# distributed-information-bottleneck/distributed-information-bottleneck.github.io

Hardware: AMD Instinct MI355X
Metric: DIB train samples/sec (fwd+KL+bwd+Adam) (higher is better)
Workload: dtype f32; 1 GPU; BASELINE config 3: synthetic tabular, 2^20 rows x 64 scalar features resident in HBM, posenc [2,4,8,16], encoder [128,128], E=32, integration [256,256], out=1, BCE-from-logits, Adam; per_gpu_batch=65536, global_batch=65536, parallelism=dp1, rccl_ranks_joined=1, dataset_rows=1048576, params=2224897

## Files before the change

distributed-information-bottleneck.github.io_amd/csrc/dib_api.hip:

```cpp
#include <algorithm>
#include <atomic>
#include <cmath>
#include <cstdio>
#include <cstdlib>
#include <cstring>
#include <map>
#include <mutex>
#include <new>
#include <utility>
#include <vector>

#include "../../include/dib_hip.h"
#include "dib_elementwise.h"
#include "dib_gauss_lse.h"
#include "dib_mi_rows.h"
#include "dib_gemm.h"
#include "dib_wgrad_stream.h"
#include "dib_infonce_mfma.h"
#include "dib_fused.h"
#include "dib_wgrad_recompute.h"
#include "dib_tail.h"
#include "dib_small.h"
#include "dib_st.h"
#include "dib_attn.h"
#include "dib_attn_small.h"
#include "dib_st_chain.h"
#include "dib_measure.h"
#include "dib_circuit.h"
#include "dib_partition.h"
#include "dib_st_info.h"
#include "dib_mi_channel.h"
#include "dib_input_grad.h"
#include "../../include/dib_st.h"
#include "../../include/dib_measure.h"
#include "../../include/dib_circuit.h"
#include "../../include/dib_partition.h"
#include "../../include/dib_mi_channel.h"

#include "host/common.h"
#include "host/layout.h"
#include "host/gemm.h"
#include "host/encoder.h"
#include "host/input_grad.h"
#include "host/small.h"
#include "host/step.h"
#include "host/infonce.h"
#include "host/st.h"
#include "host/mi.h"
#include "host/measure.h"
#include "host/circuit.h"
#include "host/partition.h"
```

distributed-information-bottleneck.github.io_amd/csrc/host/common.h:

```cpp

static std::atomic<unsigned long long> g_dib_launches{0};
#define DIB_LAUNCH(...) do { g_dib_launches.fetch_add(1, std::memory_order_relaxed); hipLaunchKernelGGL(__VA_ARGS__); } while (0)

namespace {

constexpr int64_t kAlign = 64;
constexpr int kMaxSplits = 32;
constexpr int kSmallMaxBatch = 2048;
constexpr int kSmallMaxEncWgs = 1024;
constexpr size_t kSmallMaxLds = 160 * 1024;
constexpr int kSplitRows = 512;
inline int64_t align_up(int64_t v, int64_t a = kAlign) { return (v + a - 1) / a * a; }
inline int cdiv(int64_t a, int64_t b) { return (int)((a + b - 1) / b); }
inline int grid_for(int64_t n, int per_block = 256, int cap = 256 * 16) {
  return (int)std::max<int64_t>(1, std::min<int64_t>((n + per_block - 1) / per_block, cap));
}

constexpr int kProfCats = 19;
constexpr int kProfWgradH1Part = 19;
constexpr int kProfFusedFwd = 12, kProfFusedBwd = 13, kProfOther = 14, kProfAttnFwd = 15, kProfAttnBwd = 16;
constexpr int kProfWgradStream128 = 17, kProfWgradStream64 = 18;
struct Prof {
  std::atomic<bool> on{false};
  std::mutex mu;
  std::vector<hipEvent_t> pool;
  std::vector<std::pair<hipEvent_t, hipEvent_t>> spans[kProfCats];
  std::vector<size_t> h1_spans;
  hipEvent_t get() {
    if (!pool.empty()) { hipEvent_t e = pool.back(); pool.pop_back(); return e; }
    hipEvent_t e = nullptr;
    (void)hipEventCreate(&e);
    return e;
  }
} g_prof;

struct ProfScope {
  int cat; hipStream_t st; hipEvent_t a = nullptr, b = nullptr;
  bool h1_part;
  ProfScope(int c, hipStream_t s, bool h1 = false) : cat(c), st(s), h1_part(h1) {
    if (g_prof.on.load(std::memory_order_relaxed) && cat != 14) {
      { std::lock_guard<std::mutex> lk(g_prof.mu); a = g_prof.get(); b = g_prof.get(); }
      (void)hipEventRecord(a, st);
    }
  }
  ~ProfScope() {
    if (a) {
      (void)hipEventRecord(b, st);
      std::lock_guard<std::mutex> lk(g_prof.mu);
      if (h1_part) g_prof.h1_spans.push_back(g_prof.spans[cat].size());
      g_prof.spans[cat].push_back({a, b});
    }
  }
};

const char* kVersion = "dib_hip 0.4 (gfx950: fused encoder-bank fwd/bwd + grouped fp32-MFMA GEMM + flash attention)";

int act_ok(int a) { return a >= 0 && a <= 7; }

struct Tuning {
  int fwd_small_wgs = 512;
  int fwd_narrow_wgs = 1024;
  int stream_rows = 8192;
  int split_policy = 1;
  int split_overhead = 128;
  int fused_encoder = 1;
  int fused_head = 1;
  int small_batch = 1;
  int small_wgs = 512;
  int mlp_row_tiles = 1;
  int infonce_one_launch = 1;
  int attn_small_bwd_waves = 8;
  int wgrad_flat_tile = 1;
  int wgrad_stream = 1;
  int wgrad_stream_rows = 8192;
  int wgrad_stream_fill = 85;
  int wgrad_recompute_h1 = 1;
  int attn_fwd_waves = 8;
  int int_cluster_short_exchange = 1;
  int int_cluster = 8;
  int int_cluster_wgs = 256;
  int int_cluster_min_weights = 65536;
  int wgrad_max_splits = 32;
  int num_cus = 0;
};
inline Tuning& tuning() { static Tuning t; return t; }
inline const Tuning& knobs() { return tuning(); }
inline int wgrad_max_splits() { return std::max(1, std::min(32, knobs().wgrad_max_splits)); }
inline int device_cus() {
  static std::atomic<int> cus[64];
  int dev = 0;
  if (hipGetDevice(&dev) != hipSuccess || dev < 0 || dev >= 64) return 256;
  int v = cus[dev].load(std::memory_order_relaxed);
  if (v > 0) return v;
  if (hipDeviceGetAttribute(&v, hipDeviceAttributeMultiprocessorCount, dev) != hipSuccess || v <= 0) return 256;
  cus[dev].store(v, std::memory_order_relaxed);
  return v;
}
inline int split_rule_cus() { return knobs().num_cus > 0 ? knobs().num_cus : device_cus(); }

std::mutex g_attr_mu;
template <auto* Kernel>
int raise_dynamic_lds(size_t bytes) {
  if (bytes <= 64 * 1024) return DIB_OK;
  static std::atomic<size_t> granted[64];
  int dev = 0;
  std::atomic<size_t>* slot = hipGetDevice(&dev) == hipSuccess && dev >= 0 && dev < 64 ? &granted[dev] : nullptr;
  if (slot && slot->load(std::memory_order_acquire) >= bytes) return DIB_OK;
  std::lock_guard<std::mutex> lk(g_attr_mu);
  if (slot && slot->load(std::memory_order_relaxed) >= bytes) return DIB_OK;
  hipError_t e = hipFuncSetAttribute((const void*)Kernel, hipFuncAttributeMaxDynamicSharedMemorySize, (int)bytes);
  if (e != hipSuccess) return (int)e;
  if (slot) slot->store(bytes, std::memory_order_release);
  return DIB_OK;
}
template <auto* Kernel, typename... Args>
int launch_lds(dim3 grid, dim3 block, size_t lds, hipStream_t st, Args&&... args) {
  if (int rc = raise_dynamic_lds<Kernel>(lds)) return rc;
  DIB_LAUNCH(Kernel, grid, block, lds, st, std::forward<Args>(args)...);
  return (int)hipGetLastError();
}

static int* tuning_slot(const char* key) {
  Tuning& t = tuning();
  if (!key) return nullptr;
  if (!std::strcmp(key, "fwd_small_wgs")) return &t.fwd_small_wgs;
  if (!std::strcmp(key, "fwd_narrow_wgs")) return &t.fwd_narrow_wgs;
  if (!std::strcmp(key, "stream_rows")) return &t.stream_rows;
  if (!std::strcmp(key, "split_policy")) return &t.split_policy;
  if (!std::strcmp(key, "split_overhead")) return &t.split_overhead;
  if (!std::strcmp(key, "fused_encoder")) return &t.fused_encoder;
  if (!std::strcmp(key, "fused_head")) return &t.fused_head;
  if (!std::strcmp(key, "small_batch")) return &t.small_batch;
  if (!std::strcmp(key, "small_wgs")) return &t.small_wgs;
  if (!std::strcmp(key, "mlp_row_tiles")) return &t.mlp_row_tiles;
  if (!std::strcmp(key, "infonce_one_launch")) return &t.infonce_one_launch;
  if (!std::strcmp(key, "attn_small_bwd_waves")) return &t.attn_small_bwd_waves;
  if (!std::strcmp(key, "wgrad_flat_tile")) return &t.wgrad_flat_tile;
  if (!std::strcmp(key, "wgrad_stream")) return &t.wgrad_stream;
  if (!std::strcmp(key, "wgrad_stream_rows")) return &t.wgrad_stream_rows;
  if (!std::strcmp(key, "wgrad_stream_fill")) return &t.wgrad_stream_fill;
  if (!std::strcmp(key, "wgrad_recompute_h1")) return &t.wgrad_recompute_h1;
  if (!std::strcmp(key, "wgrad_max_splits")) return &t.wgrad_max_splits;
  if (!std::strcmp(key, "num_cus")) return &t.num_cus;
  if (!std::strcmp(key, "attn_fwd_waves")) return &t.attn_fwd_waves;
  if (!std::strcmp(key, "int_cluster_short_exchange")) return &t.int_cluster_short_exchange;
  if (!std::strcmp(key, "int_cluster")) return &t.int_cluster;
  if (!std::strcmp(key, "int_cluster_wgs")) return &t.int_cluster_wgs;
  if (!std::strcmp(key, "int_cluster_min_weights")) return &t.int_cluster_min_weights;
  return nullptr;
}

}

extern "C" {

const char* dib_version(void) { return kVersion; }
int dib_abi_version(void) { return DIB_ABI_VERSION; }

const char* dib_error_string(int code) {
  switch (code) {
    case DIB_OK: return "ok";
    case DIB_E_ARG: return "invalid argument";
    case DIB_E_SHAPE: return "shape mismatch";
    case DIB_E_WORKSPACE: return "workspace / descriptor tables missing";
    case DIB_E_UNSUPPORTED: return "unsupported configuration";
    case DIB_E_NODEVICE: return "no HIP device";
    default: return code > 0 ? hipGetErrorString((hipError_t)code) : "unknown dib error";
  }
}

int dib_set_tuning(const char* key, int value) {
  int* p = tuning_slot(key);
  if (!p || value < 0) return DIB_E_ARG;
  *p = value;
  return DIB_OK;
}

int dib_get_tuning(const char* key, int* value) {
  const int* p = tuning_slot(key);
  if (!p || !value) return DIB_E_ARG;
  *value = *p;
  return DIB_OK;
}

int64_t dib_launch_count(void) { return (int64_t)g_dib_launches.load(std::memory_order_relaxed); }

int dib_profile_enable(int on) {
  std::lock_guard<std::mutex> lk(g_prof.mu);
  for (int c = 0; c < kProfCats; ++c) {
    for (auto& sp : g_prof.spans[c]) { g_prof.pool.push_back(sp.first); g_prof.pool.push_back(sp.second); }
    g_prof.spans[c].clear();
  }
  g_prof.h1_spans.clear();
  g_prof.on = on != 0;
  return DIB_OK;
}

int dib_profile_summary_n(double* ms_by_category, int* launches_by_category, int n) {
  if (!ms_by_category || !launches_by_category || n < 0) return DIB_E_ARG;
  std::lock_guard<std::mutex> lk(g_prof.mu);
  for (int c = 0; c < std::min(n, kProfCats); ++c) {
    double tot = 0.0;
    for (auto& sp : g_prof.spans[c]) {
      hipError_t e = hipEventSynchronize(sp.second);
      if (e != hipSuccess) return (int)e;
      float ms = 0.f;
      e = hipEventElapsedTime(&ms, sp.first, sp.second);
      if (e != hipSuccess) return (int)e;
      tot += ms;
    }
    ms_by_category[c] = tot;
    launches_by_category[c] = (int)g_prof.spans[c].size();
  }
  for (int c = kProfCats; c < n; ++c) { ms_by_category[c] = 0.0; launches_by_category[c] = 0; }
  if (n > kProfWgradH1Part) {
    double tot = 0.0;
    for (size_t i : g_prof.h1_spans) {
      const auto& sp = g_prof.spans[kProfWgradStream128][i];
      float ms = 0.f;
      hipError_t e = hipEventElapsedTime(&ms, sp.first, sp.second);
      if (e != hipSuccess) return (int)e;
      tot += ms;
    }
    ms_by_category[kProfWgradH1Part] = tot;
    launches_by_category[kProfWgradH1Part] = (int)g_prof.h1_spans.size();
  }
  return DIB_OK;
}

int dib_profile_summary(double* ms_by_category, int* launches_by_category) {
  return dib_profile_summary_n(ms_by_category, launches_by_category, DIB_PROFILE_CATEGORIES);
}

}
```

distributed-information-bottleneck.github.io_amd/csrc/host/gemm.h:

```cpp

namespace {

template <int MODE, int NI, int NJ, bool FLAT = false>
int launch_gemm_t(const DibGemmGroup* dev_groups, const GemmCall& c, int M, int N, const float* A, const float* B, float* C,
                  const float* bias, const float* aux, float* bias_out, int batch, int act, int nsplit,
                  int rows_per_split, long long split_stride, hipStream_t st) {
  const int tm = cdiv(M, FLAT ? 32 : 64 * NI), tn = cdiv(N, FLAT ? 256 : 64 * NJ);
  if (c.count > 65535 || (MODE == 2 && (long long)tm * tn > 65535)) return DIB_E_UNSUPPORTED;
  dim3 grid;
  if (MODE == 2) grid = dim3(nsplit, tm * tn, c.count);
  else grid = dim3(8 * cdiv(tm, 8) * tn, 1, c.count);
  constexpr int BK = FLAT ? 32 : ((NI == 2 && NJ == 2) ? 64 : ((MODE == 2 && NI == 1 && NJ == 2) ? 64 : 32));
  const long long streamed_rows = MODE == 2 ? (long long)nsplit * rows_per_split : (long long)M;
  const bool big_out = MODE != 2 && (long long)M * N * (long long)sizeof(float) * c.count >= (256ll << 20);
  const int stream_flags = streamed_rows >= knobs().stream_rows ? (big_out ? 3 : 1) : 0;
  DIB_LAUNCH((dib_gemm_kernel<MODE, NI, NJ, BK, FLAT>), grid, dim3(256), 0, st, dev_groups + c.first, A, B, C,
                     bias, aux, bias_out, batch, act, tm, tn, rows_per_split, split_stride, stream_flags);
  return (int)hipGetLastError();
}

constexpr int kWgradStreamWavesPerCu = 4;
static bool wgrad_stream_shape_ok(const DibGemmGroup* hg, int count, int batch, const float* A, const float* B, int* nt_out) {
  if (!knobs().wgrad_stream || !hg || count <= 0) return false;
  if ((((uintptr_t)A | (uintptr_t)B) & 15) != 0) return false;
  int nt = 0;
  for (int i = 0; i < count; ++i) {
    const DibGemmGroup& g = hg[i];
    const int M = g.M < 0 ? batch : g.M, N = g.N < 0 ? batch : g.N, K = g.K < 0 ? batch : g.K;
    if (M <= 0 || (M & 127) || K <= 0 || (K & 63)) return false;
    const int nt_g = N == 64 ? 2 : ((N > 0 && (N & 127) == 0) ? 4 : 0);
    if (!nt_g || (nt && nt != nt_g)) return false;
    nt = nt_g;
    if (((g.a_off + g.a_boff * batch) | (g.b_off + g.b_boff * batch) | (long long)g.lda | (long long)g.ldb) & 3) return false;
    if (g.lda < M || g.ldb < N) return false;
  }
  *nt_out = nt;
  return true;
}
static bool wgrad_stream_slabs_ok(const DibGemmGroup* hg, int count, int batch, long long tiles, int nsplit, int rows_per_split) {
  if (nsplit <= 0 || rows_per_split <= 0 || (long long)nsplit * rows_per_split < knobs().wgrad_stream_rows) return false;
  if (tiles * nsplit * 100 < (long long)knobs().wgrad_stream_fill * split_rule_cus() * kWgradStreamWavesPerCu) return false;
  for (int i = 0; i < count; ++i) {
    const int K = hg[i].K < 0 ? batch : hg[i].K;
    if ((rows_per_split & 63) && !(nsplit == 1 && rows_per_split >= K)) return false;
    if (((long long)std::min(rows_per_split, K) + 8) * std::max(hg[i].lda, hg[i].ldb) * 4 >= (1ll << 31)) return false;
  }
  return true;
}
template <int NT, int CH>
int launch_wgrad_stream(const DibGemmGroup* dev_groups, const GemmCall& c, int M, int N, const float* A, const float* B, float* C,
                        float* bias_out, int batch, int nsplit, int rows_per_split, long long split_stride, hipStream_t st) {
  const int tm = cdiv(M, 128), tn = cdiv(N, 32 * NT);
  const long long waves = (long long)tm * tn * c.count * nsplit;
  if (waves >= (1ll << 31)) return DIB_E_UNSUPPORTED;
  ProfScope ps(NT == 4 ? kProfWgradStream128 : kProfWgradStream64, st);
  const dim3 grid((unsigned)((waves + 3) / 4));
  if ((long long)nsplit * rows_per_split >= knobs().stream_rows)
    DIB_LAUNCH((dib_wgrad_stream_kernel<NT, CH, true>), grid, dim3(256), 0, st, dev_groups + c.first, A, B, C, bias_out, batch,
               c.count, tm, tn, nsplit, rows_per_split, split_stride);
  else
    DIB_LAUNCH((dib_wgrad_stream_kernel<NT, CH, false>), grid, dim3(256), 0, st, dev_groups + c.first, A, B, C, bias_out, batch,
               c.count, tm, tn, nsplit, rows_per_split, split_stride);
  return (int)hipGetLastError();
}

static void pick_wgrad_splits(long long tiles, int slots, int K, int max_splits, int* ns_out, int* rps_out) {
  const int min_rows = std::min(kSplitRows, std::max(64, *rps_out));
  const auto cost_of = [&](int ns, int rps) {
    return (double)((tiles * ns + slots - 1) / slots) * (rps + knobs().split_overhead);
  };
  {
    const long long wgs = tiles * *ns_out, rounds = (wgs + slots - 1) / slots;
    if ((double)wgs >= 0.85 * (double)(rounds * slots)) return;
  }
  double best = 1e300;
  int bns = *ns_out, brps = *rps_out;
  for (int ns = 1; ns <= max_splits; ++ns) {
    const int rps = cdiv(cdiv(K, ns), 64) * 64;
    if (ns > 1 && rps < min_rows) break;
    if (cdiv(K, rps) != ns) continue;
    const double cost = cost_of(ns, rps);
    if (cost < best) {
      best = cost;
      bns = ns;
      brps = rps;
    }
  }
  if (best >= cost_of(*ns_out, *rps_out)) return;
  *ns_out = bns;
  *rps_out = brps;
}

static void wgrad_tile_rule(int M, int N, int nsplit, int count, bool* ni1, bool* nj1) {
  *ni1 = M <= 64;
  *nj1 = N <= 64;
  if (!*ni1 && !*nj1) {
    const long long wgs = (long long)cdiv(M, 128) * cdiv(N, 128) * nsplit * count;
    if (wgs < 256) *ni1 = true;
    if (*ni1 && !*nj1 && (long long)cdiv(M, 64) * cdiv(N, 128) * nsplit * count < 128) *nj1 = true;
  }
}

struct WgradStreamPlan { int nt = 0, ch = 0, nsplit = 0, rows_per_split = 0; };
static bool wgrad_stream_plan(const DibGemmGroup* host_groups, const GemmCall& c, const float* A, const float* B, int batch, int nsplit,
                              int rows_per_split, bool auto_split, int max_splits, WgradStreamPlan* plan) {
  const int M = c.max_m < 0 ? batch : c.max_m, N = c.max_n < 0 ? batch : c.max_n;
  int nt = 0;
  if (c.count <= 0 || !wgrad_stream_shape_ok(host_groups, c.count, batch, A, B, &nt)) return false;
  int ns = nsplit, rps = rows_per_split;
  const long long tiles = (long long)cdiv(M, 128) * cdiv(N, 32 * nt) * c.count;
  if (auto_split && ns > 1 && knobs().split_policy)
    pick_wgrad_splits(tiles, split_rule_cus() * kWgradStreamWavesPerCu, batch, std::max(ns, max_splits), &ns, &rps);
  if (!wgrad_stream_slabs_ok(host_groups, c.count, batch, tiles, ns, rps)) return false;
  bool ni1, nj1;
  wgrad_tile_rule(M, N, nsplit, c.count, &ni1, &nj1);
  plan->nt = nt;
  plan->ch = nt == 2 || nj1 ? 4 : 2;
  plan->nsplit = ns;
  plan->rows_per_split = rps;
  return true;
}

template <int CH, bool RELU>
int launch_wgrad_h1_t(const DibGemmGroup* dev_groups, const DibWgradH1Side* dev_side, const GemmCall& c, int M, int N, const float* P,
                      const float* params, const float* B, float* C, float* bias_out, int batch, int nsplit, int rows_per_split,
                      long long split_stride, hipStream_t st) {
  const int tm = cdiv(M, 128), tn = cdiv(N, 128);
  const long long waves = (long long)tm * tn * c.count * nsplit;
  if (waves >= (1ll << 31)) return DIB_E_UNSUPPORTED;
  ProfScope ps(kProfWgradStream128, st, true);
  const dim3 grid((unsigned)((waves + 3) / 4));
  if ((long long)nsplit * rows_per_split >= knobs().stream_rows)
    DIB_LAUNCH((dib_wgrad_h1_kernel<CH, true, RELU>), grid, dim3(256), 0, st, dev_groups + c.first, dev_side, P, params, B, C,
               bias_out, batch, c.count, tm, tn, nsplit, rows_per_split, split_stride);
  else
    DIB_LAUNCH((dib_wgrad_h1_kernel<CH, false, RELU>), grid, dim3(256), 0, st, dev_groups + c.first, dev_side, P, params, B, C,
               bias_out, batch, c.count, tm, tn, nsplit, rows_per_split, split_stride);
  return (int)hipGetLastError();
}
static int launch_wgrad_h1(int ch, bool relu, const DibGemmGroup* dev_groups, const DibWgradH1Side* dev_side, const GemmCall& c,
                           const float* P, const float* params, const float* B, float* C, float* bias_out, int batch, int nsplit,
                           int rows_per_split, long long split_stride, hipStream_t st) {
#define DIB_GO(CH, RELU) launch_wgrad_h1_t<CH, RELU>(dev_groups, dev_side, c, c.max_m, c.max_n, P, params, B, C, bias_out, batch, nsplit, \
                                                     rows_per_split, split_stride, st)
  if (ch == 4) return relu ? DIB_GO(4, true) : DIB_GO(4, false);
  return relu ? DIB_GO(2, true) : DIB_GO(2, false);
#undef DIB_GO
}

template <int MODE>
int launch_gemm(const DibGemmGroup* dev_groups, const GemmCall& c, const float* A, const float* B, float* C,
                const float* bias, const float* aux, float* bias_out, int batch, int act, int nsplit, int rows_per_split,
                long long split_stride, hipStream_t st, bool auto_split = false, int max_splits = 0, int* ns_used = nullptr,
                const DibGemmGroup* host_groups = nullptr) {
  if (ns_used) *ns_used = nsplit;
  if (c.count == 0) return DIB_OK;
  const int M = c.max_m < 0 ? batch : c.max_m;
  const int N = c.max_n < 0 ? batch : c.max_n;
  bool ni1 = (MODE == 2) && M <= 64, nj1 = N <= 64;
  if (MODE != 2) {
    const long long wgs = (long long)cdiv(M, 128) * cdiv(N, nj1 ? 64 : 128) * c.count;
    if (wgs < knobs().fwd_small_wgs) ni1 = true;
    if (ni1 && !nj1 && (long long)cdiv(M, 64) * cdiv(N, 128) * c.count < (MODE == 0 ? knobs().fwd_narrow_wgs : 128)) nj1 = true;
  }
  if (MODE == 2) wgrad_tile_rule(M, N, nsplit, c.count, &ni1, &nj1);
  if constexpr (MODE == 2) {
    WgradStreamPlan sp;
    if (wgrad_stream_plan(host_groups, c, A, B, batch, nsplit, rows_per_split, auto_split, max_splits, &sp)) {
      const int ns = sp.nsplit, rps = sp.rows_per_split;
      if (ns_used) *ns_used = ns;
      if (sp.nt == 2) return launch_wgrad_stream<2, 4>(dev_groups, c, M, N, A, B, C, bias_out, batch, ns, rps, split_stride, st);
      return sp.ch == 4 ? launch_wgrad_stream<4, 4>(dev_groups, c, M, N, A, B, C, bias_out, batch, ns, rps, split_stride, st)
                        : launch_wgrad_stream<4, 2>(dev_groups, c, M, N, A, B, C, bias_out, batch, ns, rps, split_stride, st);
    }
  }
  if (MODE == 2 && auto_split && nsplit > 1 && knobs().split_policy) {
    const int per_cu = (!ni1 && !nj1) ? 2 : ((!ni1 && nj1) ? 4 : (ni1 && !nj1) ? 3 : 4);
    const long long tiles = (long long)cdiv(M, ni1 ? 64 : 128) * cdiv(N, nj1 ? 64 : 128) * c.count;
    pick_wgrad_splits(tiles, split_rule_cus() * per_cu, batch, std::max(nsplit, max_splits), &nsplit, &rows_per_split);
    if (ns_used) *ns_used = nsplit;
  }
  ProfScope ps(MODE * 4 + (ni1 ? 0 : 2) + (nj1 ? 0 : 1), st);
  if constexpr (MODE == 2) {
    if (M <= 32 && N >= 256 && knobs().wgrad_flat_tile)
      return launch_gemm_t<2, 1, 2, true>(dev_groups, c, M, N, A, B, C, bias, aux, bias_out, batch, act, nsplit, rows_per_split,
                                          split_stride, st);
  }
#define DIB_GO(NI, NJ) launch_gemm_t<MODE, NI, NJ>(dev_groups, c, M, N, A, B, C, bias, aux, bias_out, batch, act, nsplit, \
                                                   rows_per_split, split_stride, st)
  if (ni1) return nj1 ? DIB_GO(1, 1) : DIB_GO(1, 2);
  return nj1 ? DIB_GO(2, 1) : DIB_GO(2, 2);
#undef DIB_GO
}

__global__ void dib_write_desc_kernel(DibGemmGroup* dst, DibGemmGroup g) { *dst = g; }

static int retire_stale_slabs(const dib_layout* l, int batch, const DibGemmGroup* host_groups, int count, int ns, int slab_count,
                              float* gt, long long split_stride, hipStream_t st) {
  hipStreamCaptureStatus cap = hipStreamCaptureStatusNone;
  const bool capturing = hipStreamIsCapturing(st, &cap) == hipSuccess && cap == hipStreamCaptureStatusActive;
  std::lock_guard<std::mutex> lk(l->wg_mu);
  for (int i = 0; i < count; ++i) {
    const DibGemmGroup& g = host_groups[i];
    int& mark = l->slab_hwm[std::make_pair(batch, g.c_off)];
    mark = std::max(mark, ns);
    const int hwm = capturing ? std::max(mark, slab_count) : mark;
    if (ns >= hwm) continue;
    const size_t wbytes = (size_t)g.M * (size_t)g.ldc * sizeof(float);
    for (int s = ns; s < hwm; ++s) {
      hipError_t e = hipMemsetAsync(gt + (long long)s * split_stride + g.c_off, 0, wbytes, st);
      if (e == hipSuccess && g.bias_off >= 0)
        e = hipMemsetAsync(gt + (long long)s * split_stride + g.bias_off, 0, (size_t)g.N * sizeof(float), st);
      if (e != hipSuccess) return (int)e;
    }
  }
  return DIB_OK;
}

template <int MODE>
int launch_gemm(const dib_layout* l, const GemmCall& c, const float* A, const float* B, float* C, const float* bias,
                const float* aux, float* bias_out, int batch, int act, int nsplit, int rows_per_split,
                long long split_stride, hipStream_t st, int slab_count = 0) {
  int ns_used = nsplit;
  int rc = launch_gemm<MODE>(l->dev_groups, c, A, B, C, bias, aux, bias_out, batch, act, nsplit, rows_per_split, split_stride,
                             st, MODE == 2, slab_count, &ns_used, MODE == 2 ? l->table.data() + c.first : nullptr);
  if (MODE == 2 && rc == DIB_OK && slab_count > 1)
    rc = retire_stale_slabs(l, batch, l->table.data() + c.first, c.count, ns_used, slab_count, C, split_stride, st);
  return rc;
}

}

static int merged_wgrad(dib_layout* l, const dib_layout::WsMap& m, float* w, int batch, float* gt, int first, int count,
                        hipStream_t st) {
  if (count <= 0) return DIB_OK;
  const auto& host = wg_table_host(l, m, batch);
  GemmCall c;
  c.first = 0; c.count = count;
  for (int i = first; i < first + count; ++i) { c.max_m = std::max(c.max_m, host[i].M); c.max_n = std::max(c.max_n, host[i].N); }
  const DibGemmGroup* dev = reinterpret_cast<const DibGemmGroup*>(w + m.wg_table) + first;
  int ns_used = m.nsplit;
  int rc = launch_gemm<2>(dev, c, w, w, gt, nullptr, nullptr, gt, batch, 0, m.nsplit, m.rows_per_split, align_up(l->n_params, 4), st,
                          true, m.nsplit, &ns_used, host.data() + first);
  if (rc == DIB_OK && m.nsplit > 1)
    rc = retire_stale_slabs(l, batch, host.data() + first, count, ns_used, m.nsplit, gt, align_up(l->n_params, 4), st);
  return rc;
}

extern "C" {

int dib_gemm(int mode, int M, int N, int K, const float* A, int lda, const float* B, int ldb, float* C, int ldc,
             const float* bias, const float* aux, int ldaux, int act, void* dev_desc, dib_stream_t stream) {
  if (!A || !B || !C || !dev_desc || M <= 0 || N <= 0 || K <= 0 || mode < 0 || mode > 2) return DIB_E_ARG;
  hipStream_t st = (hipStream_t)stream;
  DibGemmGroup g = make_group(Off(), lda, Off(), ldb, Off(), ldc, bias ? 0 : -1, Off(), ldaux, M, N, K);
  if ((((uintptr_t)A | (uintptr_t)B) & 15) != 0) return DIB_E_ARG;
  DIB_LAUNCH(dib_write_desc_kernel, dim3(1), dim3(1), 0, st, (DibGemmGroup*)dev_desc, g);
  if (hipError_t e = hipGetLastError(); e != hipSuccess) return (int)e;
  const int tm = cdiv(M, 128), tn = cdiv(N, 128);
  const DibGemmGroup* dg = (const DibGemmGroup*)dev_desc;
  const dim3 g1(8 * cdiv(tm, 8) * tn, 1, 1);
  if (mode == 0)
    DIB_LAUNCH((dib_gemm_kernel<0, 2, 2, 32>), g1, dim3(256), 0, st, dg, A, B, C, bias, aux, (float*)nullptr, 0,
                       act, tm, tn, 0, 0ll);
  else if (mode == 1)
    DIB_LAUNCH((dib_gemm_kernel<1, 2, 2, 32>), g1, dim3(256), 0, st, dg, A, B, C, bias, aux, (float*)nullptr, 0,
                       act, tm, tn, 0, 0ll);
  else
    DIB_LAUNCH((dib_gemm_kernel<2, 2, 2, 32>), dim3(1, tm * tn, 1), dim3(256), 0, st, dg, A, B, C,
                       (const float*)nullptr, aux, (float*)bias, 0, act, tm, tn, K, 0ll);
  return (int)hipGetLastError();
}

static_assert(sizeof(dib_gemm_desc) == sizeof(DibGemmGroup), "public descriptor must mirror the kernel's group struct");

int dib_gemm_grouped(int mode, int n_groups, const dib_gemm_desc* dev_desc, int max_m, int max_n, const float* A,
                     const float* B, float* C, const float* bias, const float* aux, float* bias_out, int act, int nsplit,
                     int rows_per_split, int64_t split_stride, dib_stream_t stream) {
  if (!dev_desc || !A || !B || !C || n_groups <= 0 || max_m <= 0 || max_n <= 0 || mode < 0 || mode > 2 || !act_ok(act))
    return DIB_E_ARG;
  if (mode == 2 && (nsplit <= 0 || rows_per_split <= 0)) return DIB_E_ARG;
  GemmCall c;
  c.first = 0; c.count = n_groups; c.max_m = max_m; c.max_n = max_n;
  const DibGemmGroup* g = reinterpret_cast<const DibGemmGroup*>(dev_desc);
  hipStream_t st = (hipStream_t)stream;
  switch (mode) {
    case 0: return launch_gemm<0>(g, c, A, B, C, bias, aux, nullptr, 0, act, 1, 0, 0, st);
    case 1: return launch_gemm<1>(g, c, A, B, C, nullptr, aux, nullptr, 0, act, 1, 0, 0, st);
    default: return launch_gemm<2>(g, c, A, B, C, nullptr, nullptr, bias_out, 0, 0, nsplit, rows_per_split,
                                   (long long)split_stride, st);
  }
}

int dib_wgrad_grouped(int n_groups, const dib_gemm_desc* dev_desc, const dib_gemm_desc* host_desc, int max_m, int max_n, int batch,
                      const float* A, const float* B, float* C, float* bias_out, int nsplit, int rows_per_split,
                      int64_t split_stride, dib_stream_t stream) {
  if (!dev_desc || !host_desc || !A || !B || !C || n_groups <= 0 || max_m <= 0 || max_n <= 0 || batch < 0 || nsplit <= 0 ||
      rows_per_split <= 0)
    return DIB_E_ARG;
  GemmCall c;
  c.first = 0; c.count = n_groups; c.max_m = max_m; c.max_n = max_n;
  return launch_gemm<2>(reinterpret_cast<const DibGemmGroup*>(dev_desc), c, A, B, C, nullptr, nullptr, bias_out, batch, 0, nsplit,
                        rows_per_split, (long long)split_stride, (hipStream_t)stream, false, 0, nullptr,
                        reinterpret_cast<const DibGemmGroup*>(host_desc));
}

int dib_gemm_skinny_k(int mode, int n_groups, const dib_gemm_desc* dev_desc, int M, int N, int K, const float* A,
                      const float* B, float* C, const float* bias, dib_stream_t stream) {
  if (!dev_desc || !A || !B || !C || n_groups <= 0 || M <= 0 || N <= 0 || K <= 0 || mode < 0 || mode > 1) return DIB_E_ARG;
  if (K > 32 || (K & 3) || (N & 31) || n_groups > 65535 || cdiv(N, 128) > 65535) return DIB_E_UNSUPPORTED;
  const DibGemmGroup* g = reinterpret_cast<const DibGemmGroup*>(dev_desc);
  const int total_tiles = cdiv(M, 64), cn = cdiv(N, 128);
  int chunks = std::max(1, std::min(total_tiles, cdiv(4096, cn * n_groups)));
  int tiles = std::min(8, cdiv(total_tiles, chunks));
  chunks = cdiv(total_tiles, tiles);
  const int nt_store = (long long)M * N * (long long)sizeof(float) * n_groups >= (256ll << 20) ? 1 : 0;
  const dim3 grid(chunks, cn, n_groups);
  hipStream_t st = (hipStream_t)stream;
  if (mode == 0)
    DIB_LAUNCH(dib_gemm_skinnyk_kernel<0>, grid, dim3(256), 0, st, g, A, B, C, bias, M, N, K, tiles, nt_store);
  else
    DIB_LAUNCH(dib_gemm_skinnyk_kernel<1>, grid, dim3(256), 0, st, g, A, B, C, (const float*)nullptr, M, N, K, tiles,
                       nt_store);
  return (int)hipGetLastError();
}

int dib_reduce_splits(const float* partial, int64_t n, int nsplit, int64_t stride, float* out, dib_stream_t stream) {
  if (!partial || !out || n <= 0 || nsplit <= 0 || (n & 3) || (stride & 3)) return DIB_E_ARG;
  DIB_LAUNCH(dib_reduce_splits_kernel, dim3(grid_for(n / 4)), dim3(256), 0, (hipStream_t)stream, partial,
                     (long long)n, nsplit, (long long)stride, out, (const float*)nullptr);
  return (int)hipGetLastError();
}

int dib_reduce_splits_add(const float* partial, int64_t n, int nsplit, int64_t stride, float* out, dib_stream_t stream) {
  if (!partial || !out || n <= 0 || nsplit <= 0 || (n & 3) || (stride & 3)) return DIB_E_ARG;
  DIB_LAUNCH(dib_reduce_splits_kernel, dim3(grid_for(n / 4)), dim3(256), 0, (hipStream_t)stream, partial,
                     (long long)n, nsplit, (long long)stride, out, (const float*)out);
  return (int)hipGetLastError();
}

}
```

include/dib_hip.h:

```cpp
#ifndef DIB_HIP_H
#define DIB_HIP_H

#include <stdint.h>

#ifdef __cplusplus
extern "C" {
#endif

typedef struct dib_layout dib_layout;
typedef void* dib_stream_t;

#define DIB_OK 0
#define DIB_E_ARG (-1)
#define DIB_E_SHAPE (-2)
#define DIB_E_WORKSPACE (-3)
#define DIB_E_UNSUPPORTED (-4)
#define DIB_E_NODEVICE (-5)

enum { DIB_ACT_LINEAR = 0, DIB_ACT_RELU = 1, DIB_ACT_LEAKY_RELU = 2, DIB_ACT_TANH = 3,
       DIB_ACT_SIGMOID = 4, DIB_ACT_ELU = 5, DIB_ACT_SOFTPLUS = 6 };

enum { DIB_LOSS_BCE_LOGITS = 0, DIB_LOSS_BCE = 1, DIB_LOSS_SPARSE_CCE_LOGITS = 2, DIB_LOSS_MSE = 3 };

enum { DIB_WS_U = 0,
       DIB_WS_PRED = 1,
       DIB_WS_ENC_OUT = 2,
       DIB_WS_G_U = 3,
       DIB_WS_STEP_OUT = 4,
       DIB_WS_G_PRED = 5,
       DIB_WS_ENC_H0 = 16,
       DIB_WS_INT_H0 = 32    };

const char* dib_version(void);
#define DIB_ABI_VERSION 7
int dib_abi_version(void);
const char* dib_error_string(int code);

int dib_layout_create(int num_features, const int* feature_dims, int n_enc_layers, const int* enc_units,
                      int embedding_dim, int n_int_layers, const int* int_units, int output_dim,
                      int use_positional_encoding, int n_freq, int activation, int output_activation,
                      dib_layout** out);
void dib_layout_destroy(dib_layout* l);
int64_t dib_layout_param_count(const dib_layout* l);
int dib_layout_param_block(const dib_layout* l, int net, int layer, int feature, int what, int64_t* offset,
                           int* rows, int* cols);
int64_t dib_layout_table_bytes(const dib_layout* l);
int dib_layout_upload_tables(dib_layout* l, void* dev_tables, dib_stream_t stream);
int dib_layout_set_step_counter(dib_layout* l, const uint32_t* step_dev);
int64_t dib_workspace_bytes(const dib_layout* l, int batch);
int dib_workspace_init(const dib_layout* l, int batch, void* ws, dib_stream_t stream);
int64_t dib_workspace_offset(const dib_layout* l, int batch, int which);
int dib_layout_wgrad_splits(const dib_layout* l, int batch);
int dib_workspace_h1_stashed(const dib_layout* l, const void* ws);
int dib_workspace_h1_materialize(dib_layout* l, int batch, const float* params, void* ws, dib_stream_t stream);

#define DIB_FWD_DETERMINISTIC 1
#define DIB_FWD_INFERENCE 2
#define DIB_FWD_DEFER_SUMS 4
int dib_encoder_bank_fwd(dib_layout* l, const float* x, int64_t ldx, const int32_t* row_idx, int64_t row0,
                         int batch, const float* params, uint64_t seed, uint32_t step, int deterministic,
                         void* ws, dib_stream_t stream);
int dib_integration_fwd(dib_layout* l, int batch, const float* params, void* ws, dib_stream_t stream);

#define DIB_HEAD_DEFER_SUMS 1
#define DIB_HEAD_NO_GRAD 2
#define DIB_HEAD_DEFER_WGRAD 4
int dib_loss_fwd_bwd(dib_layout* l, int loss_kind, const float* y, int64_t ldy, const int32_t* row_idx,
                     int64_t row0, int batch, float inv_global_batch, int flags, void* ws, dib_stream_t stream);
int dib_integration_bwd(dib_layout* l, int batch, const float* params, float* grads, void* ws,
                        dib_stream_t stream);
int dib_output_head_fused_supported(const dib_layout* l, int loss_kind);
int dib_integration_fwd_hidden(dib_layout* l, int batch, const float* params, void* ws, dib_stream_t stream);
int dib_output_head_fused(dib_layout* l, int loss_kind, const float* y, int64_t ldy, const int32_t* row_idx, int64_t row0,
                          int batch, float inv_global_batch, int flags, const float* params, float* grads, void* ws,
                          dib_stream_t stream);
int dib_integration_bwd_hidden(dib_layout* l, int batch, const float* params, float* grads, void* ws,
                               dib_stream_t stream);
int dib_integration_head_step(dib_layout* l, int loss_kind, const float* y, int64_t ldy, const int32_t* row_idx, int64_t row0,
                              int batch, float inv_global_batch, int flags, const float* params, float* grads, void* ws,
                              dib_stream_t stream);
#define DIB_BWD_INTEGRATION_DONE 1
int dib_backward(dib_layout* l, int batch, const float* params, float* grads, const float* beta_dev, float inv_global_batch,
                 int flags, void* ws, dib_stream_t stream);
int dib_encoder_bank_bwd(dib_layout* l, int batch, const float* params, float* grads, const float* beta_dev,
                         float inv_global_batch, void* ws, dib_stream_t stream);
int dib_encoder_bank_input_grad(dib_layout* l, const float* x, int64_t ldx, const int32_t* row_idx, int64_t row0, int batch,
                                const float* params, void* ws, float* dx, int64_t lddx, dib_stream_t stream);
int dib_encoder_bank_bwd_stage(dib_layout* l, int batch, const float* params, float* grads, const float* beta_dev,
                               float inv_global_batch, int stage, void* ws, dib_stream_t stream);
int dib_grads_finalize(dib_layout* l, int batch, float* grads, void* ws, dib_stream_t stream);
int dib_grads_finalize_part(dib_layout* l, int batch, int part, float* grads, void* ws, dib_stream_t stream);
int dib_layout_part_range(const dib_layout* l, int part, int64_t* offset, int64_t* count);
int dib_metrics_accumulate(dib_layout* l, int batch, const float* beta_dev, float inv_global_batch,
                           float* metrics_acc, void* ws, dib_stream_t stream);
#define DIB_TAIL_FINALIZE 1
#define DIB_TAIL_KL 2
#define DIB_TAIL_LOSS 4
#define DIB_TAIL_ADAM 8
#define DIB_TAIL_BUMP 16
#define DIB_TAIL_METRICS 32
#define DIB_TAIL_SGD 64
#define DIB_TAIL_HEAD_WGRAD 128
#define DIB_TAIL_LOSS_HEAD 256
int dib_step_tail(dib_layout* l, int batch, int part, int flags, float* params, float* grads, float* adam_m, float* adam_v,
                  const float* lr_dev, int64_t* t_dev, float beta1, float beta2, float eps, float grad_scale,
                  const float* beta_dev, float inv_global_batch, float* metrics_acc, void* ws, dib_stream_t stream);

int dib_set_tuning(const char* key, int value);
int dib_get_tuning(const char* key, int* value);

int dib_adam_step(float* params, const float* grads, float* m, float* v, int64_t n, const float* lr_dev,
                  int64_t* t_dev, float beta1, float beta2, float eps, float grad_scale, dib_stream_t stream);
int dib_sgd_step(float* params, const float* grads, int64_t n, const float* lr_dev, float grad_scale,
                 dib_stream_t stream);
#define DIB_SYNC_WORDS 1056
int dib_reduce_adam_step(const float* partial, int nsplit, int64_t stride, float* params, float* grads, float* adam_m,
                         float* adam_v, int64_t n, const float* lr_dev, int64_t* t_dev, float beta1, float beta2, float eps,
                         float grad_scale, uint32_t* sync, dib_stream_t stream);

int dib_encode_deterministic(dib_layout* l, int feature, const float* x_f, int n, const float* params,
                             float* out, void* ws, dib_stream_t stream);
int dib_bhattacharyya(const float* mu1, const float* lv1, int n, const float* mu2, const float* lv2, int m,
                      int dim, float* out, dib_stream_t stream);
int64_t dib_infonce_workspace_bytes(int batch);
int dib_infonce_fwd_bwd(const float* emb_x, const float* emb_y, int batch, int dim, int similarity, float temperature,
                        float* g_x, float* g_y, float* loss_out, void* ws, dib_stream_t stream);
int dib_positional_encoding(const float* x, int64_t ldx, int n, int d, int n_freq, float* out, dib_stream_t stream);
int dib_positional_encoding_rows(const float* x, int64_t ldx, const int32_t* row_idx, int n, int d, int n_freq, float* out,
                                 dib_stream_t stream);

typedef struct dib_mlp_desc {
  int64_t w_off[4], b_off[4];
  int32_t n_hidden, width[4];
  int32_t in_dim, n_freq, act;
} dib_mlp_desc;
int dib_mlp_small_supported(const dib_mlp_desc* d, int batch);
int dib_mlp_small_fwd(const dib_mlp_desc* d, const float* params, const float* x, int64_t ldx, const int32_t* row_idx, int n,
                      float* a0, float* const* h, float* out, dib_stream_t stream);
int dib_mlp_small_bwd(const dib_mlp_desc* d, const float* params, const float* g_out, float* const* h, float* const* g, int n,
                      dib_stream_t stream);
int dib_mlp_small_head_supported(const dib_mlp_desc* d, int n);
int64_t dib_mlp_small_head_workspace_bytes(const dib_mlp_desc* d, int n);
int dib_mlp_small_head_step(const dib_mlp_desc* d, const float* params, const float* x, int n, const float* y, int64_t ldy,
                            int loss_kind, float inv_global_batch, float* const* h, float* const* g, float* pred, float* g_pred,
                            float* g_x, float* grads, float* sums3, void* ws, dib_stream_t stream);
int dib_integration_fwd_and_mlp_fwd(dib_layout* l, int batch, const float* params, void* ws, const dib_mlp_desc* d,
                                    const float* mlp_params, const float* x, int64_t ldx, const int32_t* row_idx, int n, float* a0,
                                    float* const* h, float* out, dib_stream_t stream);
int dib_backward_and_mlp_bwd(dib_layout* l, int batch, const float* params, float* grads, const float* beta_dev,
                             float inv_global_batch, int flags, void* ws, const dib_mlp_desc* d, const float* mlp_params,
                             const float* g_out, float* const* h, float* const* g, int n, dib_stream_t stream);

int64_t dib_mi_workspace_bytes(int n, int embedding_dim);
int dib_mi_sandwich_rows(const float* enc_out, int n, int embedding_dim, uint64_t seed, uint32_t step,
                         uint32_t feature, double* lower_rows, double* upper_rows, void* ws, dib_stream_t stream);
int dib_philox_normal_fill(float* eps, const int32_t* row_idx, int64_t row0, int batch, int num_features,
                           int embedding_dim, uint64_t seed, uint32_t step, dib_stream_t stream);
float dib_philox_normal_ref(uint64_t seed, uint32_t step, uint32_t row, uint32_t feature, uint32_t e);

int64_t dib_launch_count(void);
#define DIB_PROFILE_CATEGORIES 17
int dib_profile_enable(int on);
int dib_profile_summary(double* ms_by_category , int* launches_by_category );
#define DIB_PROFILE_CATEGORIES_N 20
int dib_profile_summary_n(double* ms_by_category , int* launches_by_category , int n);

int dib_gemm(int mode, int M, int N, int K, const float* A, int lda, const float* B, int ldb, float* C,
             int ldc, const float* bias, const float* aux, int ldaux, int act, void* dev_desc ,
             dib_stream_t stream);

#ifdef __cplusplus
}
#endif
#endif
```

Measured before the change: 8.201 million samples/s.

## Add register-streamed persistent MFMA GEMM for large forward and dgrad calls

Adds a persistent kernel for forward and dgrad GEMMs. Each wave owns a contiguous range of 128x128 output tiles, keeps A and B fragments in registers without LDS, and software-pipelines the global loads of the next K-slab and next tile under the fp32 MFMAs. Bias, ReLU/leaky activation and the dgrad activation mask are applied in the epilogue, with optional nontemporal stores for large outputs. It is chosen when M is at least 8192 rows, the shape and alignment constraints hold, and there are enough tiles to fill the waves. The aim is to cut LDS staging, barriers and tile-launch overhead on the large-batch GEMMs, at the cost of very high register pressure (one wave per SIMD) and a reliance on cache reuse for B.

```diff
diff --git a/distributed-information-bottleneck.github.io_amd/csrc/dib_api.hip b/distributed-information-bottleneck.github.io_amd/csrc/dib_api.hip
--- a/distributed-information-bottleneck.github.io_amd/csrc/dib_api.hip
+++ b/distributed-information-bottleneck.github.io_amd/csrc/dib_api.hip
@@ -15,6 +15,7 @@
 #include "dib_gauss_lse.h"
 #include "dib_mi_rows.h"
 #include "dib_gemm.h"
+#include "dib_gemm_stream.h"
 #include "dib_wgrad_stream.h"
 #include "dib_infonce_mfma.h"
 #include "dib_fused.h"
diff --git a/distributed-information-bottleneck.github.io_amd/csrc/dib_gemm_stream.h b/distributed-information-bottleneck.github.io_amd/csrc/dib_gemm_stream.h
--- /dev/null
+++ b/distributed-information-bottleneck.github.io_amd/csrc/dib_gemm_stream.h
@@ -0,0 +1,178 @@
+#pragma once
+#include "dib_gemm.h"
+
+typedef float dib_gs_f4 __attribute__((ext_vector_type(4)));
+typedef float dib_gs_f2 __attribute__((ext_vector_type(2)));
+
+__device__ __forceinline__ dib_gs_f4 dib_gs_load(const char* p) { return *reinterpret_cast<const dib_gs_f4*>(p); }
+
+template <int MODE, int KIND>
+__global__ void __launch_bounds__(256, 1)
+dib_gemm_stream_kernel(const DibGemmGroup* __restrict__ groups, const float* __restrict__ Abase, const float* __restrict__ Bbase,
+                       float* __restrict__ Cbase, const float* __restrict__ bias, const float* __restrict__ aux, int batch, int act,
+                       int tiles_m, int tiles_n, int nwaves, int nts) {
+  static_assert((MODE == 0 && KIND >= 0 && KIND <= 2) || (MODE == 1 && (KIND == 0 || KIND == 3)), "forward and dgrad; the weight gradient is dib_wgrad_stream.h");
+  typedef dib_gs_f4 f4v;
+  typedef dib_gs_f2 f2v;
+  const int lane = threadIdx.x & 63, l31 = lane & 31, h = lane >> 5;
+  const unsigned wave = (unsigned)__builtin_amdgcn_readfirstlane((int)(threadIdx.x >> 6));
+  const unsigned nwg = gridDim.x, wg = blockIdx.x;
+  const unsigned v = ((nwg & 7u) == 0u ? (wg & 7u) * (nwg >> 3) + (wg >> 3) : wg) * 4u + wave;
+  if (v >= (unsigned)nwaves) return;
+  const unsigned tiles = (unsigned)tiles_m * (unsigned)tiles_n;
+  unsigned tile = (unsigned)((unsigned long long)v * tiles / (unsigned)nwaves);
+  const unsigned tend = (unsigned)((unsigned long long)(v + 1u) * tiles / (unsigned)nwaves);
+  if (tile >= tend) return;
+  const DibGemmGroup g = groups[0];
+  const int K = g.K < 0 ? batch : g.K;
+  const int nsb = K >> 5;
+
+  const char* Ag = reinterpret_cast<const char*>(Abase + g.a_off + g.a_boff * batch);
+  const char* Bg = reinterpret_cast<const char*>(Bbase + g.b_off + g.b_boff * batch);
+  const unsigned rowA = (unsigned)g.lda * 4u, rowB = (unsigned)g.ldb * 4u, subA = 32u * rowA;
+  const unsigned laneA = (unsigned)l31 * rowA + 16u * (unsigned)h;
+  const unsigned laneB = MODE == 0 ? 4u * (unsigned)h * rowB + 16u * (unsigned)l31 : 4u * (unsigned)l31 * rowB + 16u * (unsigned)h;
+  auto a_base = [&](unsigned t) { return Ag + (size_t)(t / (unsigned)tiles_n) * 128u * (size_t)rowA + (size_t)laneA; };
+  auto b_base = [&](unsigned t) {
+    const size_t n0 = (size_t)(t % (unsigned)tiles_n) * 128u;
+    return Bg + (MODE == 0 ? n0 * 4u : n0 * (size_t)rowB) + (size_t)laneB;
+  };
+
+  f4v a[4][4];
+  f4v bw1[4][4];
+  f2v bw0[2][4][4];
+  auto load_a = [&](int i, const char* p, unsigned sb) {
+#pragma unroll
+    for (int q = 0; q < 4; ++q)
+      a[i][q] = dib_gs_load(p + (size_t)((unsigned)i * subA + 128u * sb) + 32 * q);
+  };
+  auto load_b = [&](int jp, int hf, const char* p, unsigned sb) {
+    if (MODE == 1) {
+#pragma unroll
+      for (int q = 0; q < 4; ++q)
+        bw1[2 * jp + hf][q] = dib_gs_load(p + (size_t)((unsigned)(2 * jp + hf) * rowB + 128u * sb) + 32 * q);
+    } else {
+#pragma unroll
+      for (int qq = 0; qq < 2; ++qq)
+#pragma unroll
+        for (int t = 0; t < 4; ++t)
+          bw0[jp][2 * hf + qq][t] = *reinterpret_cast<const f2v*>(p + (size_t)((32u * sb + (unsigned)(8 * (2 * hf + qq) + t)) * rowB) + 8 * jp);
+    }
+  };
+
+  const char* pA = a_base(tile);
+  const char* pB = b_base(tile);
+  load_b(0, 0, pB, 0u);
+  __builtin_amdgcn_sched_barrier(0);
+  load_a(0, pA, 0u);
+  __builtin_amdgcn_sched_barrier(0);
+  load_b(0, 1, pB, 0u);
+  __builtin_amdgcn_sched_barrier(0);
+  load_a(1, pA, 0u);
+  __builtin_amdgcn_sched_barrier(0);
+  load_a(2, pA, 0u);
+  __builtin_amdgcn_sched_barrier(0);
+
+  char* Cg = reinterpret_cast<char*>(Cbase + g.c_off + g.c_boff * batch);
+  const char* auxg = KIND == 3 ? reinterpret_cast<const char*>(aux + g.aux_off + g.aux_boff * batch) : nullptr;
+  const unsigned rowC = (unsigned)g.ldc * 4u, rowX = (unsigned)g.ldaux * 4u;
+  const float slope = act == 1 ? 0.0f : (act == 2 ? 0.2f : (act == 7 ? 0.1f : 1.0f));
+  const unsigned laneC = 4u * (unsigned)h * rowC + 16u * (unsigned)l31, laneX = 4u * (unsigned)h * rowX + 16u * (unsigned)l31;
+
+#pragma unroll 1
+  for (; tile < tend; ++tile) {
+    const unsigned tnext = min(tile + 1u, tend - 1u);
+    const bool more = tile + 1u < tend;
+    const char* pA1 = a_base(tnext);
+    const char* pB1 = b_base(tnext);
+    dib_f32x16 acc[4][4];
+#pragma unroll
+    for (int i = 0; i < 4; ++i)
+#pragma unroll
+      for (int j = 0; j < 4; ++j)
+#pragma unroll
+        for (int r = 0; r < 16; ++r) acc[i][j][r] = 0.f;
+    int S = 0;
+#pragma unroll 1
+    do {
+      const bool last = S + 1 == nsb;
+      const char* pAn = last ? pA1 : pA;
+      const char* pBn = last ? pB1 : pB;
+      const unsigned Sn = last ? (more ? 0u : (unsigned)S) : (unsigned)S + 1u;
+#pragma unroll
+      for (int ph = 0; ph < 8; ++ph) {
+        const int jp = ph >> 2, i = ph & 3;
+#pragma unroll
+        for (int q = 0; q < 4; ++q) {
+#pragma unroll
+          for (int t = 0; t < 4; ++t) {
+#pragma unroll
+            for (int jj = 0; jj < 2; ++jj) {
+              const int j = 2 * jp + jj;
+              acc[i][j] = DIB_MFMA(a[i][q][t], MODE == 0 ? bw0[jp][q][t][jj] : bw1[j][q][t], acc[i][j]);
+            }
+            const int step = 4 * q + t;
+            const bool la = step == 0 && (ph == 0 || ph >= 5);
+            const bool lb = (step == 4 && (ph == 0 || ph == 1 || ph == 4 || ph == 5));
+            if (la || lb) {
+              __builtin_amdgcn_sched_barrier(0);
+              if (la) {
+                if (ph == 0) load_a(3, pA, (unsigned)S);
+                else load_a(ph - 5, pAn, Sn);
+              } else {
+                if (ph < 2) load_b(1, ph, pB, (unsigned)S);
+                else load_b(0, ph - 4, pBn, Sn);
+              }
+              __builtin_amdgcn_sched_barrier(0);
+            }
+          }
+        }
+      }
+    } while (++S < nsb);
+
+    const size_t m0 = (size_t)(tile / (unsigned)tiles_n) * 128u, n0 = (size_t)(tile % (unsigned)tiles_n) * 128u;
+    char* cp = Cg + m0 * rowC + n0 * 4u + (size_t)laneC;
+    f4v bv = 0.f;
+    if (MODE == 0 && bias != nullptr && g.bias_off >= 0) {
+      const float* bp = bias + g.bias_off + n0 + 4 * l31;
+      bv = f4v{bp[0], bp[1], bp[2], bp[3]};
+    }
+    const char* xp = KIND == 3 ? auxg + m0 * rowX + n0 * 4u + (size_t)laneX : nullptr;
+#pragma unroll
+    for (int i = 0; i < 4; ++i) {
+#pragma unroll
+      for (int rg = 0; rg < 4; ++rg) {
+        f4v x[4], o[4];
+        if (KIND == 3) {
+#pragma unroll
+          for (int rr = 0; rr < 4; ++rr) x[rr] = dib_gs_load(xp + (size_t)((unsigned)(32 * i + 8 * rg + rr) * rowX));
+        }
+#pragma unroll
+        for (int rr = 0; rr < 4; ++rr) {
+          const int r = 4 * rg + rr;
+          o[rr] = f4v{acc[i][0][r], acc[i][1][r], acc[i][2][r], acc[i][3][r]};
+          if (MODE == 0) o[rr] += bv;
+          if (MODE == 1 && KIND == 0) asm volatile("" : "+v"(o[rr]));
+#pragma unroll
+          for (int j = 0; j < 4; ++j) {
+            if (KIND == 1) o[rr][j] = fmaxf(o[rr][j], 0.0f);
+            else if (KIND == 2) o[rr][j] = o[rr][j] > 0.0f ? o[rr][j] : slope * o[rr][j];
+            else if (KIND == 3) o[rr][j] *= x[rr][j] > 0.0f ? 1.0f : slope;
+          }
+        }
+        if (nts) {
+#pragma unroll
+          for (int rr = 0; rr < 4; ++rr)
+            __builtin_nontemporal_store(o[rr], reinterpret_cast<f4v*>(cp + (size_t)((unsigned)(32 * i + 8 * rg + rr) * rowC)));
+        } else {
+#pragma unroll
+          for (int rr = 0; rr < 4; ++rr)
+            *reinterpret_cast<f4v*>(cp + (size_t)((unsigned)(32 * i + 8 * rg + rr) * rowC)) = o[rr];
+        }
+        __builtin_amdgcn_sched_barrier(0);
+      }
+    }
+    pA = pA1;
+    pB = pB1;
+  }
+}
diff --git a/distributed-information-bottleneck.github.io_amd/csrc/host/common.h b/distributed-information-bottleneck.github.io_amd/csrc/host/common.h
--- a/distributed-information-bottleneck.github.io_amd/csrc/host/common.h
+++ b/distributed-information-bottleneck.github.io_amd/csrc/host/common.h
@@ -18,6 +18,7 @@
 
 constexpr int kProfCats = 19;
 constexpr int kProfWgradH1Part = 19;
+constexpr int kProfGemmStreamPart = 20;
 constexpr int kProfFusedFwd = 12, kProfFusedBwd = 13, kProfOther = 14, kProfAttnFwd = 15, kProfAttnBwd = 16;
 constexpr int kProfWgradStream128 = 17, kProfWgradStream64 = 18;
 struct Prof {
@@ -26,6 +27,7 @@
   std::vector<hipEvent_t> pool;
   std::vector<std::pair<hipEvent_t, hipEvent_t>> spans[kProfCats];
   std::vector<size_t> h1_spans;
+  std::vector<size_t> gs_spans[2];
   hipEvent_t get() {
     if (!pool.empty()) { hipEvent_t e = pool.back(); pool.pop_back(); return e; }
     hipEvent_t e = nullptr;
@@ -37,7 +39,8 @@
 struct ProfScope {
   int cat; hipStream_t st; hipEvent_t a = nullptr, b = nullptr;
   bool h1_part;
-  ProfScope(int c, hipStream_t s, bool h1 = false) : cat(c), st(s), h1_part(h1) {
+  int gs_mode;
+  ProfScope(int c, hipStream_t s, bool h1 = false, int gs = -1) : cat(c), st(s), h1_part(h1), gs_mode(gs) {
     if (g_prof.on.load(std::memory_order_relaxed) && cat != 14) {
       { std::lock_guard<std::mutex> lk(g_prof.mu); a = g_prof.get(); b = g_prof.get(); }
       (void)hipEventRecord(a, st);
@@ -48,6 +51,7 @@
       (void)hipEventRecord(b, st);
       std::lock_guard<std::mutex> lk(g_prof.mu);
       if (h1_part) g_prof.h1_spans.push_back(g_prof.spans[cat].size());
+      if (gs_mode >= 0) g_prof.gs_spans[gs_mode].push_back(g_prof.spans[cat].size());
       g_prof.spans[cat].push_back({a, b});
     }
   }
@@ -74,6 +78,9 @@
   int wgrad_stream = 1;
   int wgrad_stream_rows = 8192;
   int wgrad_stream_fill = 85;
+  int gemm_stream = 1;
+  int gemm_stream_rows = 8192;
+  int gemm_stream_fill = 85;
   int wgrad_recompute_h1 = 1;
   int attn_fwd_waves = 8;
   int int_cluster_short_exchange = 1;
@@ -139,6 +146,9 @@
   if (!std::strcmp(key, "wgrad_stream")) return &t.wgrad_stream;
   if (!std::strcmp(key, "wgrad_stream_rows")) return &t.wgrad_stream_rows;
   if (!std::strcmp(key, "wgrad_stream_fill")) return &t.wgrad_stream_fill;
+  if (!std::strcmp(key, "gemm_stream")) return &t.gemm_stream;
+  if (!std::strcmp(key, "gemm_stream_rows")) return &t.gemm_stream_rows;
+  if (!std::strcmp(key, "gemm_stream_fill")) return &t.gemm_stream_fill;
   if (!std::strcmp(key, "wgrad_recompute_h1")) return &t.wgrad_recompute_h1;
   if (!std::strcmp(key, "wgrad_max_splits")) return &t.wgrad_max_splits;
   if (!std::strcmp(key, "num_cus")) return &t.num_cus;
@@ -192,6 +202,8 @@
     g_prof.spans[c].clear();
   }
   g_prof.h1_spans.clear();
+  g_prof.gs_spans[0].clear();
+  g_prof.gs_spans[1].clear();
   g_prof.on = on != 0;
   return DIB_OK;
 }
@@ -225,6 +237,18 @@
     ms_by_category[kProfWgradH1Part] = tot;
     launches_by_category[kProfWgradH1Part] = (int)g_prof.h1_spans.size();
   }
+  for (int mode = 0; mode < 2 && n > kProfGemmStreamPart + mode; ++mode) {
+    double tot = 0.0;
+    for (size_t i : g_prof.gs_spans[mode]) {
+      const auto& sp = g_prof.spans[mode * 4 + 3][i];
+      float ms = 0.f;
+      hipError_t e = hipEventElapsedTime(&ms, sp.first, sp.second);
+      if (e != hipSuccess) return (int)e;
+      tot += ms;
+    }
+    ms_by_category[kProfGemmStreamPart + mode] = tot;
+    launches_by_category[kProfGemmStreamPart + mode] = (int)g_prof.gs_spans[mode].size();
+  }
   return DIB_OK;
 }
 
diff --git a/distributed-information-bottleneck.github.io_amd/csrc/host/gemm.h b/distributed-information-bottleneck.github.io_amd/csrc/host/gemm.h
--- a/distributed-information-bottleneck.github.io_amd/csrc/host/gemm.h
+++ b/distributed-information-bottleneck.github.io_amd/csrc/host/gemm.h
@@ -61,6 +61,55 @@
   else
     DIB_LAUNCH((dib_wgrad_stream_kernel<NT, CH, false>), grid, dim3(256), 0, st, dev_groups + c.first, A, B, C, bias_out, batch,
                c.count, tm, tn, nsplit, rows_per_split, split_stride);
+  return (int)hipGetLastError();
+}
+
+struct GemmStreamPlan { int tiles_m = 0, tiles_n = 0, nwaves = 0, kind = 0; };
+static bool gemm_stream_plan(int mode, const DibGemmGroup* hg, const GemmCall& c, const float* A, const float* B, const float* C,
+                             const float* bias, const float* aux, int batch, int act, GemmStreamPlan* plan) {
+  if (!knobs().gemm_stream || !hg || c.count != 1 || (mode != 0 && mode != 1)) return false;
+  if (!(act == 0 || act == 1 || act == 2 || act == 7)) return false;
+  const DibGemmGroup& g = hg[0];
+  const long long M = g.M < 0 ? batch : g.M, N = g.N < 0 ? batch : g.N, K = g.K < 0 ? batch : g.K;
+  if (M <= 0 || (M & 127) || N <= 0 || (N & 127) || K <= 0 || (K & 31)) return false;
+  if (M < knobs().gemm_stream_rows) return false;
+  const bool mask = mode == 1 && aux != nullptr && act != 0;
+  if ((((uintptr_t)A | (uintptr_t)B | (uintptr_t)C | (mask ? (uintptr_t)aux : 0)) & 15) != 0) return false;
+  if (((g.a_off + g.a_boff * batch) | (g.b_off + g.b_boff * batch) | (g.c_off + g.c_boff * batch) | (long long)g.lda | (long long)g.ldb |
+       (long long)g.ldc) & 3)
+    return false;
+  if (mask && (((g.aux_off + g.aux_boff * batch) | (long long)g.ldaux) & 3)) return false;
+  if (g.lda < K || g.ldb < (mode == 0 ? N : K) || g.ldc < N || (mask && g.ldaux < N)) return false;
+  const long long ext = std::max({128ll * g.lda, (mode == 0 ? K : 128ll) * g.ldb, 128ll * g.ldc, mask ? 128ll * g.ldaux : 0ll});
+  if ((ext + 8) * 4 >= (1ll << 31)) return false;
+  const long long tm = M / 128, tn = N / 128, tiles = tm * tn;
+  if (tiles >= (1ll << 31)) return false;
+  const long long slots = (long long)split_rule_cus() * kWgradStreamWavesPerCu;
+  if (tiles * 100 < (long long)knobs().gemm_stream_fill * slots) return false;
+  plan->tiles_m = (int)tm;
+  plan->tiles_n = (int)tn;
+  plan->nwaves = (int)std::min(tiles, slots);
+  plan->kind = mode == 0 ? (act == 0 ? 0 : (act == 1 ? 1 : 2)) : (mask ? 3 : 0);
+  return true;
+}
+template <int MODE>
+int launch_gemm_stream(const GemmStreamPlan& sp, const DibGemmGroup* dev_group, const DibGemmGroup& hg, const float* A, const float* B,
+                       float* C, const float* bias, const float* aux, int batch, int act, hipStream_t st) {
+  ProfScope ps(MODE * 4 + 3, st, false, MODE);
+  const long long M = hg.M < 0 ? batch : hg.M, N = hg.N < 0 ? batch : hg.N;
+  const int nts = M >= knobs().stream_rows && M * N * (long long)sizeof(float) >= (256ll << 20) ? 1 : 0;
+  const dim3 grid((unsigned)((sp.nwaves + 3) / 4));
+#define DIB_GO(KIND) DIB_LAUNCH((dib_gemm_stream_kernel<MODE, KIND>), grid, dim3(256), 0, st, dev_group, A, B, C, bias, aux, batch, act, \
+                                sp.tiles_m, sp.tiles_n, sp.nwaves, nts)
+  if constexpr (MODE == 0) {
+    if (sp.kind == 1) DIB_GO(1);
+    else if (sp.kind == 0) DIB_GO(0);
+    else DIB_GO(2);
+  } else {
+    if (sp.kind == 3) DIB_GO(3);
+    else DIB_GO(0);
+  }
+#undef DIB_GO
   return (int)hipGetLastError();
 }
 
@@ -164,6 +213,11 @@
     if (ni1 && !nj1 && (long long)cdiv(M, 64) * cdiv(N, 128) * c.count < (MODE == 0 ? knobs().fwd_narrow_wgs : 128)) nj1 = true;
   }
   if (MODE == 2) wgrad_tile_rule(M, N, nsplit, c.count, &ni1, &nj1);
+  if constexpr (MODE != 2) {
+    GemmStreamPlan gp;
+    if (gemm_stream_plan(MODE, host_groups, c, A, B, C, bias, aux, batch, act, &gp))
+      return launch_gemm_stream<MODE>(gp, dev_groups + c.first, host_groups[0], A, B, C, bias, aux, batch, act, st);
+  }
   if constexpr (MODE == 2) {
     WgradStreamPlan sp;
     if (wgrad_stream_plan(host_groups, c, A, B, batch, nsplit, rows_per_split, auto_split, max_splits, &sp)) {
@@ -223,7 +277,7 @@
                 long long split_stride, hipStream_t st, int slab_count = 0) {
   int ns_used = nsplit;
   int rc = launch_gemm<MODE>(l->dev_groups, c, A, B, C, bias, aux, bias_out, batch, act, nsplit, rows_per_split, split_stride,
-                             st, MODE == 2, slab_count, &ns_used, MODE == 2 ? l->table.data() + c.first : nullptr);
+                             st, MODE == 2, slab_count, &ns_used, l->table.data() + c.first);
   if (MODE == 2 && rc == DIB_OK && slab_count > 1)
     rc = retire_stale_slabs(l, batch, l->table.data() + c.first, c.count, ns_used, slab_count, C, split_stride, st);
   return rc;
@@ -259,6 +313,15 @@
   if (hipError_t e = hipGetLastError(); e != hipSuccess) return (int)e;
   const int tm = cdiv(M, 128), tn = cdiv(N, 128);
   const DibGemmGroup* dg = (const DibGemmGroup*)dev_desc;
+  if (mode != 2) {
+    GemmCall c;
+    c.first = 0; c.count = 1; c.max_m = M; c.max_n = N;
+    GemmStreamPlan gp;
+    if (gemm_stream_plan(mode, &g, c, A, B, C, bias, aux, 0, act, &gp))
+      return mode == 0 ? launch_gemm_stream<0>(gp, dg, g, A, B, C, bias, aux, 0, act, st)
+                       : launch_gemm_stream<1>(gp, dg, g, A, B, C, bias, aux, 0, act, st);
+  }
+  ProfScope ps(mode * 4 + 3, st);
   const dim3 g1(8 * cdiv(tm, 8) * tn, 1, 1);
   if (mode == 0)
     DIB_LAUNCH((dib_gemm_kernel<0, 2, 2, 32>), g1, dim3(256), 0, st, dg, A, B, C, bias, aux, (float*)nullptr, 0,
diff --git a/include/dib_hip.h b/include/dib_hip.h
--- a/include/dib_hip.h
+++ b/include/dib_hip.h
@@ -162,7 +162,7 @@
 #define DIB_PROFILE_CATEGORIES 17
 int dib_profile_enable(int on);
 int dib_profile_summary(double* ms_by_category , int* launches_by_category );
-#define DIB_PROFILE_CATEGORIES_N 20
+#define DIB_PROFILE_CATEGORIES_N 22
 int dib_profile_summary_n(double* ms_by_category , int* launches_by_category , int n);
 
 int dib_gemm(int mode, int M, int N, int K, const float* A, int lda, const float* B, int ldb, float* C,
```

After: 8.634 million samples/s (median of 6 runs). 5.3% higher.
